# mr3543/3d-Object-Detection

Measured on AMD Instinct MI355X. Metric: lidar sweeps/sec end-to-end fwd (pillarize+backbone), 60k pts, 500×500 BEV, higher is better.
Workload: dtype f32

## Files before the change

### 3d-object-detection_amd/csrc/pp_conv_split.hip

```cpp

#include <algorithm>

#include "pp_conv_split.h"
#include "pp_conv_train.h"
#include "pp_conv_split_tile.h"

namespace pp {

namespace {

using G = TileGeo<8, 1, 1, 2>;

}

template <bool BARE>
__global__ __launch_bounds__(256, 1) void k_conv3x3_split(const float *__restrict__ x,
                                                          const uint4 *__restrict__ w,
                                                          const float *__restrict__ esc,
                                                          const float *__restrict__ prm,
                                                          float *__restrict__ y, int H, int W, int Cin,
                                                          int64_t y_stride, int tiles_x, int tiles_y) {
  __shared__ __attribute__((aligned(16))) unsigned char lds[2 * G::kBufBytes];

  const int lane = threadIdx.x & 63, wave = threadIdx.x >> 6;
  int bx, by, b;
  tile_of_block(tiles_x, tiles_y, bx, by, b);
  const int oy0 = by * G::kRows, ox0 = bx * kTw;
  const int co0 = blockIdx.y * kCo;
  const int nchunks = Cin / kKc;
  Stager<G, BARE> stage(x, w, b, H, W, Cin, oy0 - 1, ox0 - 1, nchunks);
  if constexpr (BARE) stage.xs = prm ? prm[0] : 1.0f;

  const int h = lane >> 5, l32 = lane & 31;
  const int a_off = h * G::kAPlane + (2 * wave * G::kHw + l32) * 16;
  const int b_off = G::kABytes + (h * kCo + l32) * 16;

  f32x16 m00 = {}, m01 = {}, m10 = {}, m11 = {}, c00 = {}, c01 = {}, c10 = {}, c11 = {};

  auto mfmas = [&](const unsigned char *cur) {
#pragma unroll
    for (int dy = 0; dy < 3; ++dy)
#pragma unroll
      for (int dx = 0; dx < 3; ++dx) {
        const int tap = 3 * dy + dx;
        const unsigned char *pa = cur + a_off + (dy * G::kHw + dx) * 16;
        const unsigned char *pb = cur + b_off + tap * (2 * kCo * 16);
        const f16x8 a0h = *reinterpret_cast<const f16x8 *>(pa);
        const f16x8 a1h = *reinterpret_cast<const f16x8 *>(pa + G::kHw * 16);
        const f16x8 b0h = *reinterpret_cast<const f16x8 *>(pb);
        const f16x8 b1h = *reinterpret_cast<const f16x8 *>(pb + 32 * 16);
        const f16x8 b0l = *reinterpret_cast<const f16x8 *>(pb + G::kBPart);
        const f16x8 b1l = *reinterpret_cast<const f16x8 *>(pb + G::kBPart + 32 * 16);
        const f16x8 a0l = *reinterpret_cast<const f16x8 *>(pa + G::kAPart);
        const f16x8 a1l = *reinterpret_cast<const f16x8 *>(pa + G::kAPart + G::kHw * 16);
        m00 = __builtin_amdgcn_mfma_f32_32x32x16_f16(a0h, b0h, m00, 0, 0, 0);
        m01 = __builtin_amdgcn_mfma_f32_32x32x16_f16(a0h, b1h, m01, 0, 0, 0);
        m10 = __builtin_amdgcn_mfma_f32_32x32x16_f16(a1h, b0h, m10, 0, 0, 0);
        m11 = __builtin_amdgcn_mfma_f32_32x32x16_f16(a1h, b1h, m11, 0, 0, 0);
        c00 = __builtin_amdgcn_mfma_f32_32x32x16_f16(a0h, b0l, c00, 0, 0, 0);
        c01 = __builtin_amdgcn_mfma_f32_32x32x16_f16(a0h, b1l, c01, 0, 0, 0);
        c10 = __builtin_amdgcn_mfma_f32_32x32x16_f16(a1h, b0l, c10, 0, 0, 0);
        c11 = __builtin_amdgcn_mfma_f32_32x32x16_f16(a1h, b1l, c11, 0, 0, 0);
        c00 = __builtin_amdgcn_mfma_f32_32x32x16_f16(a0l, b0h, c00, 0, 0, 0);
        c01 = __builtin_amdgcn_mfma_f32_32x32x16_f16(a0l, b1h, c01, 0, 0, 0);
        c10 = __builtin_amdgcn_mfma_f32_32x32x16_f16(a1l, b0h, c10, 0, 0, 0);
        c11 = __builtin_amdgcn_mfma_f32_32x32x16_f16(a1l, b1h, c11, 0, 0, 0);
      }
  };

  chunk_pipeline(stage, lds, nchunks, mfmas);

  const int co = co0 + l32;
  const float e0 = esc[co], e1 = esc[co + 32];
  const auto ep = [&] {
    if constexpr (BARE)
      return Unscale{prm ? prm[1] : 1.0f};
    else
      return Epilogue<2>(prm, co);
  }();
#pragma unroll
  for (int m = 0; m < 2; ++m) {
    const int oy = oy0 + 2 * wave + m;
    if (oy >= H) continue;
    float *yrow = y + (((int64_t)b * H + oy) * W + ox0) * y_stride + co;
    const f32x16 v0 = m ? m10 : m00, v1 = m ? m11 : m01, d0 = m ? c10 : c00, d1 = m ? c11 : c01;
#pragma unroll
    for (int r = 0; r < 16; ++r) {
      const int px = (r & 3) + 8 * (r >> 2) + 4 * h;
      if (ox0 + px < W) {
        float *yp = yrow + px * y_stride;
        yp[0] = split_output<BARE>(v0[r], d0[r], e0, ep, 0);
        yp[32] = split_output<BARE>(v1[r], d1[r], e1, ep, 1);
      }
    }
  }
}

}

using namespace pp;

template <bool BARE>
static int conv3x3_split(const char *fn, pp_ctx_t *ctx, void *stream_, const float *x_dev, int batch, int height,
                         int width, int in_channels, const void *w_split_dev, int out_channels, const float *prm,
                         float *y_dev, int64_t y_channels, int64_t y_channel_offset) {
  if (int rc = check_conv_f16_args(fn, ctx, x_dev, w_split_dev, BARE ? x_dev : prm, y_dev, batch, height, width,
                                   in_channels, out_channels, y_channels, y_channel_offset))
    return rc;
  const int64_t tiles_x = (width + kTw - 1) / kTw, tiles_y = (height + G::kRows - 1) / G::kRows;
  const int64_t blocks = (int64_t)batch * tiles_x * tiles_y;
  if (blocks > 0x7fffffff ||
      (int64_t)batch * height * width * std::max<int64_t>(in_channels, y_channels) > ((int64_t)1 << 40)) {
    set_error("%s: tensor too large", fn);
    return PP_ERR_VALUE;
  }
  const uint4 *w = static_cast<const uint4 *>(w_split_dev);
  const float *esc = split_scales(w_split_dev, out_channels, in_channels);
  return launch_on_device(ctx, "k_conv3x3_split", [&] {
    hipLaunchKernelGGL(k_conv3x3_split<BARE>, dim3((unsigned)blocks, (unsigned)(out_channels / 64)), dim3(256), 0,
                       static_cast<hipStream_t>(stream_), x_dev, w, esc, prm, y_dev + y_channel_offset, height, width,
                       in_channels, y_channels, (int)tiles_x, (int)tiles_y);
  });
}

extern "C" int pp_conv3x3_split_nhwc_dev(pp_ctx_t *ctx, void *stream_, const float *x_dev, int batch,
                                         int height, int width, int in_channels, const void *w_split_dev,
                                         int out_channels, const float *params_dev, float *y_dev,
                                         int64_t y_channels, int64_t y_channel_offset) {
  return conv3x3_split<false>("pp_conv3x3_split_nhwc_dev", ctx, stream_, x_dev, batch, height, width, in_channels,
                              w_split_dev, out_channels, params_dev, y_dev, y_channels, y_channel_offset);
}

extern "C" int pp_conv3x3_split_bare_nhwc_dev(pp_ctx_t *ctx, void *stream_, const float *x_dev, int batch,
                                              int height, int width, int in_channels, const void *w_split_dev,
                                              int out_channels, const float *x_scale_dev, float *y_dev,
                                              int64_t y_channels, int64_t y_channel_offset) {
  if (reinterpret_cast<uintptr_t>(x_scale_dev) & 3) {
    set_error("pp_conv3x3_split_bare_nhwc_dev: x_scale_dev is not 4-byte aligned");
    return PP_ERR_VALUE;
  }
  return conv3x3_split<true>("pp_conv3x3_split_bare_nhwc_dev", ctx, stream_, x_dev, batch, height, width,
                             in_channels, w_split_dev, out_channels, x_scale_dev, y_dev, y_channels,
                             y_channel_offset);
}
```

Before: 2357.

## Make split conv3x3 persistent with software-pipelined loads interleaved among MFMAs

Turns the split-precision 3x3 conv kernel into a persistent kernel whose grid is capped at the compute-unit count, so each block walks over (tile, output-group) items. Each step interleaves the 108 MFMAs with LDS fragment reads, direct global-to-LDS weight DMA, and the f32→f16 hi/lo conversion of the next chunk's activations, and it prefetches the next item's first chunk while the current item finishes. This is meant to hide load latency and launch/tail costs that the previous one-block-per-tile pipeline exposed. In exchange it relies on hand-written inline asm, explicit vmcnt waits and sched barriers, which are fragile. With one block per CU it may also leave less latency hiding across blocks.

Result: faster. 2556, median of 6 (+8.4%).

```diff
diff --git a/3d-object-detection_amd/csrc/pp_conv_split.hip b/3d-object-detection_amd/csrc/pp_conv_split.hip
--- a/3d-object-detection_amd/csrc/pp_conv_split.hip
+++ b/3d-object-detection_amd/csrc/pp_conv_split.hip
@@ -1,5 +1,7 @@
 
 #include <algorithm>
+#include <type_traits>
+#include <utility>
 
 #include "pp_conv_split.h"
 #include "pp_conv_train.h"
@@ -10,6 +12,130 @@
 namespace {
 
 using G = TileGeo<8, 1, 1, 2>;
+
+typedef __attribute__((address_space(3))) void *lptr_t;
+typedef float f32x4 __attribute__((ext_vector_type(4)));
+typedef unsigned u32x4 __attribute__((ext_vector_type(4)));
+typedef _Float16 f16x2 __attribute__((ext_vector_type(2)));
+
+constexpr int kTapMfmas = 12;
+constexpr int kStepMfmas = 9 * kTapMfmas;
+constexpr int kElems = 8 * G::kNItem;
+constexpr int kFirstSlot = kStepMfmas - 2 * kElems - 1;
+constexpr int kWavePieces = G::kWVecs / 64 / 4;
+static_assert(G::kWVecs % 256 == 0 && kFirstSlot >= kTapMfmas, "whole pieces; the conversion fits in a step");
+
+template <int... I, class F>
+__device__ __forceinline__ void static_for_impl(std::integer_sequence<int, I...>, F &&f) {
+  (f(std::integral_constant<int, I>{}), ...);
+}
+template <int N, class F>
+__device__ __forceinline__ void static_for(F &&f) {
+  static_for_impl(std::make_integer_sequence<int, N>{}, f);
+}
+
+struct Item {
+  int b, oy0, ox0, group;
+  __device__ __forceinline__ Item(int item, int groups, int tiles_x, int tiles_y) {
+    group = item % groups;
+    const int tile = item / groups;
+    ox0 = tile % tiles_x * kTw;
+    const int rest = tile / tiles_x;
+    oy0 = rest % tiles_y * G::kRows;
+    b = rest / tiles_y;
+  }
+};
+
+__device__ __forceinline__ void dma_piece(const uint4 *src, unsigned dst, unsigned lane16) {
+  unsigned keep;
+  asm volatile("s_mov_b32 %0, m0\n\ts_mov_b32 m0, %2\n\ts_nop 0\n\tglobal_load_lds_dwordx4 %1, %3\n\ts_mov_b32 m0, %0"
+               : "=&s"(keep)
+               : "v"(lane16), "s"(dst), "s"(src)
+               : "memory");
+}
+
+template <bool XS>
+struct SplitLoader {
+  static constexpr int kN = G::kNItem;
+  const int tid = threadIdx.x;
+  float xs = 1.0f;
+  const float *xb;
+  int xoff[kN], adst[kN];
+  bool xin[kN];
+  const bool last_item = tid + 256 * (kN - 1) < G::kItems;
+  f32x4 xr[kN][2];
+  u32x4 vh[kN], vl[kN];
+  unsigned eh, el;
+
+  __device__ __forceinline__ SplitLoader() {
+#pragma unroll
+    for (int k = 0; k < kN; ++k) {
+      const int i = tid + 256 * k;
+      const int pix = i >> 1, hy = pix / G::kHw;
+      adst[k] = (i & 1) * G::kAPlane + G::slot(pix, hy, pix - hy * G::kHw) * 16;
+    }
+  }
+
+  __device__ __forceinline__ void place(const float *x, const Item &it, int H, int W, int Cin) {
+    xb = x + (int64_t)it.b * H * W * Cin;
+#pragma unroll
+    for (int k = 0; k < kN; ++k) {
+      const int i = tid + 256 * k;
+      const int pix = i >> 1, hh = i & 1;
+      const int hy = pix / G::kHw, hx = pix - hy * G::kHw;
+      const int iy = it.oy0 - G::kHl + hy, ix = it.ox0 - G::kHl + hx;
+      xin[k] = i < G::kItems && iy >= 0 && iy < H && ix >= 0 && ix < W;
+      xoff[k] = (xin[k] ? (iy * W + ix) * Cin : 0) + 8 * hh;
+    }
+  }
+
+  __device__ __forceinline__ void load(int chunk) {
+    const float *xc = xb + chunk * kKc;
+#pragma unroll
+    for (int k = 0; k < kN; ++k) {
+      const float *p = xc + xoff[k];
+      asm volatile("global_load_dwordx4 %0, %2, off\n\tglobal_load_dwordx4 %1, %2, off offset:16"
+                   : "=&v"(xr[k][0]), "=&v"(xr[k][1])
+                   : "v"(p)
+                   : "memory");
+    }
+  }
+
+  template <int K, int kYounger>
+  __device__ __forceinline__ void arrived() {
+    asm volatile("s_waitcnt vmcnt(%2)" : "+v"(xr[K][0]), "+v"(xr[K][1]) : "n"(kYounger + 2 * (kN - 1 - K)));
+  }
+
+  template <int K, int J>
+  __device__ __forceinline__ void convert() {
+    asm volatile("" : "+v"(xr[K][J >> 2]));
+    float a = xr[K][J >> 2][J & 3];
+    if constexpr (XS) a = a * xs;
+    const _Float16 ah = (_Float16)a, al = (_Float16)((a - (float)ah) * 2048.0f);
+    if constexpr (J % 2 == 0) {
+      eh = __builtin_bit_cast(unsigned short, ah);
+      el = __builtin_bit_cast(unsigned short, al);
+      asm volatile("" : "+v"(eh), "+v"(el));
+    } else {
+      unsigned uh = eh | (unsigned)__builtin_bit_cast(unsigned short, ah) << 16;
+      unsigned ul = el | (unsigned)__builtin_bit_cast(unsigned short, al) << 16;
+      asm volatile("" : "+v"(uh), "+v"(ul));
+      vh[K][J >> 1] = uh;
+      vl[K][J >> 1] = ul;
+    }
+  }
+
+  template <int K>
+  __device__ __forceinline__ void write(unsigned char *buf) const {
+    u32x4 r = vl[K], v = vh[K];
+    if (!xin[K]) r = u32x4{};
+    if (!xin[K]) v = u32x4{};
+    if (K + 1 < kN || last_item) {
+      *reinterpret_cast<u32x4 *>(buf + G::kAPart + adst[K]) = r;
+      *reinterpret_cast<u32x4 *>(buf + adst[K]) = v;
+    }
+  }
+};
 
 }
 
@@ -19,80 +145,164 @@
                                                           const float *__restrict__ esc,
                                                           const float *__restrict__ prm,
                                                           float *__restrict__ y, int H, int W, int Cin,
-                                                          int64_t y_stride, int tiles_x, int tiles_y) {
+                                                          int64_t y_stride, int tiles_x, int tiles_y, int groups,
+                                                          int items) {
   __shared__ __attribute__((aligned(16))) unsigned char lds[2 * G::kBufBytes];
 
-  const int lane = threadIdx.x & 63, wave = threadIdx.x >> 6;
-  int bx, by, b;
-  tile_of_block(tiles_x, tiles_y, bx, by, b);
-  const int oy0 = by * G::kRows, ox0 = bx * kTw;
-  const int co0 = blockIdx.y * kCo;
+  const int lane = threadIdx.x & 63, wave = __builtin_amdgcn_readfirstlane(threadIdx.x >> 6);
   const int nchunks = Cin / kKc;
-  Stager<G, BARE> stage(x, w, b, H, W, Cin, oy0 - 1, ox0 - 1, nchunks);
-  if constexpr (BARE) stage.xs = prm ? prm[0] : 1.0f;
+  const int walk = gridDim.x;
+  int item = blockIdx.x;
+
+  SplitLoader<BARE> ld;
+  float inv = 1.0f;
+  if constexpr (BARE)
+    if (prm) {
+      ld.xs = prm[0];
+      inv = prm[1];
+    }
 
   const int h = lane >> 5, l32 = lane & 31;
   const int a_off = h * G::kAPlane + (2 * wave * G::kHw + l32) * 16;
   const int b_off = G::kABytes + (h * kCo + l32) * 16;
 
-  f32x16 m00 = {}, m01 = {}, m10 = {}, m11 = {}, c00 = {}, c01 = {}, c10 = {}, c11 = {};
-
-  auto mfmas = [&](const unsigned char *cur) {
-#pragma unroll
-    for (int dy = 0; dy < 3; ++dy)
-#pragma unroll
-      for (int dx = 0; dx < 3; ++dx) {
-        const int tap = 3 * dy + dx;
-        const unsigned char *pa = cur + a_off + (dy * G::kHw + dx) * 16;
-        const unsigned char *pb = cur + b_off + tap * (2 * kCo * 16);
-        const f16x8 a0h = *reinterpret_cast<const f16x8 *>(pa);
-        const f16x8 a1h = *reinterpret_cast<const f16x8 *>(pa + G::kHw * 16);
-        const f16x8 b0h = *reinterpret_cast<const f16x8 *>(pb);
-        const f16x8 b1h = *reinterpret_cast<const f16x8 *>(pb + 32 * 16);
-        const f16x8 b0l = *reinterpret_cast<const f16x8 *>(pb + G::kBPart);
-        const f16x8 b1l = *reinterpret_cast<const f16x8 *>(pb + G::kBPart + 32 * 16);
-        const f16x8 a0l = *reinterpret_cast<const f16x8 *>(pa + G::kAPart);
-        const f16x8 a1l = *reinterpret_cast<const f16x8 *>(pa + G::kAPart + G::kHw * 16);
-        m00 = __builtin_amdgcn_mfma_f32_32x32x16_f16(a0h, b0h, m00, 0, 0, 0);
-        m01 = __builtin_amdgcn_mfma_f32_32x32x16_f16(a0h, b1h, m01, 0, 0, 0);
-        m10 = __builtin_amdgcn_mfma_f32_32x32x16_f16(a1h, b0h, m10, 0, 0, 0);
-        m11 = __builtin_amdgcn_mfma_f32_32x32x16_f16(a1h, b1h, m11, 0, 0, 0);
-        c00 = __builtin_amdgcn_mfma_f32_32x32x16_f16(a0h, b0l, c00, 0, 0, 0);
-        c01 = __builtin_amdgcn_mfma_f32_32x32x16_f16(a0h, b1l, c01, 0, 0, 0);
-        c10 = __builtin_amdgcn_mfma_f32_32x32x16_f16(a1h, b0l, c10, 0, 0, 0);
-        c11 = __builtin_amdgcn_mfma_f32_32x32x16_f16(a1h, b1l, c11, 0, 0, 0);
-        c00 = __builtin_amdgcn_mfma_f32_32x32x16_f16(a0l, b0h, c00, 0, 0, 0);
-        c01 = __builtin_amdgcn_mfma_f32_32x32x16_f16(a0l, b1h, c01, 0, 0, 0);
-        c10 = __builtin_amdgcn_mfma_f32_32x32x16_f16(a1l, b0h, c10, 0, 0, 0);
-        c11 = __builtin_amdgcn_mfma_f32_32x32x16_f16(a1l, b1h, c11, 0, 0, 0);
-      }
+  f32x16 acc[8];
+  f16x8 fr[2][8];
+
+  const unsigned lds_addr = (unsigned)(uintptr_t)(lptr_t)lds;
+  const unsigned lane16 = lane * 16;
+  const int wpiece0 = G::kABytes + wave * (kWavePieces * 1024);
+  auto wpieces = [&](int group, int chunk) {
+    return w + ((int64_t)group * nchunks + chunk) * G::kWVecs + wave * (kWavePieces * 64);
   };
 
-  chunk_pipeline(stage, lds, nchunks, mfmas);
-
-  const int co = co0 + l32;
-  const float e0 = esc[co], e1 = esc[co + 32];
-  const auto ep = [&] {
-    if constexpr (BARE)
-      return Unscale{prm ? prm[1] : 1.0f};
+  auto read_frag = [&](const unsigned char *cur, auto tap_, auto f_) __attribute__((always_inline)) {
+    constexpr int tap = decltype(tap_)::value, f = decltype(f_)::value;
+    constexpr int a = (tap / 3 * G::kHw + tap % 3) * 16, b = tap * (2 * kCo * 16);
+    constexpr int off = f == 0 ? a : f == 1 ? a + G::kHw * 16 : f == 2 ? b : f == 3 ? b + 32 * 16 : f == 4 ? b + G::kBPart
+                        : f == 5 ? b + G::kBPart + 32 * 16 : f == 6 ? a + G::kAPart : a + G::kAPart + G::kHw * 16;
+    fr[tap & 1][f] = *reinterpret_cast<const f16x8 *>(cur + ((f < 2 || f >= 6) ? a_off : b_off) + off);
+  };
+
+  int par = 0;
+  auto step = [&](int ngroup, int nchunk, auto first_, auto more_) __attribute__((always_inline)) {
+    constexpr bool first = decltype(first_)::value, more = decltype(more_)::value;
+    const unsigned char *cur = lds + par * G::kBufBytes;
+    unsigned char *nxt = lds + (par ^ 1) * G::kBufBytes;
+    static_for<8>([&](auto f) { read_frag(cur, std::integral_constant<int, 0>{}, f); });
+    if constexpr (more) ld.load(nchunk);
+    const uint4 *wsrc = wpieces(ngroup, nchunk);
+    const unsigned wdst = lds_addr + (par ^ 1) * G::kBufBytes + wpiece0;
+    __builtin_amdgcn_sched_barrier(0);
+    static_for<kStepMfmas>([&](auto m_) {
+      constexpr int m = decltype(m_)::value, tap = m / kTapMfmas, i = m % kTapMfmas, s = tap & 1;
+      constexpr int ia = (i < 8 ? 0 : 6) + ((i >> 1) & 1), ib = (i >= 4 && i < 8 ? 4 : 2) + (i & 1);
+      constexpr int ic = (i < 4 ? 0 : 4) + (i & 3);
+      if constexpr (first && m < 8)
+        acc[ic] = __builtin_amdgcn_mfma_f32_32x32x16_f16(fr[s][ia], fr[s][ib], f32x16{}, 0, 0, 0);
+      else
+        acc[ic] = __builtin_amdgcn_mfma_f32_32x32x16_f16(fr[s][ia], fr[s][ib], acc[ic], 0, 0, 0);
+      __builtin_amdgcn_sched_barrier(0);
+      if constexpr (tap + 1 < 9 && i < 8) {
+        read_frag(cur, std::integral_constant<int, tap + 1>{}, std::integral_constant<int, i>{});
+        __builtin_amdgcn_sched_barrier(0);
+      }
+      if constexpr (more && m < kWavePieces) {
+        dma_piece(wsrc + m * 64, wdst + m * 1024, lane16);
+        __builtin_amdgcn_sched_barrier(0);
+      }
+      if constexpr (more && m >= kFirstSlot) {
+        constexpr int j = m - kFirstSlot, e = j / 2;
+        if constexpr (j % 2 == 0 && e < kElems) {
+          if constexpr (e % 8 == 0) ld.template arrived<e / 8, kWavePieces>();
+          ld.template convert<e / 8, e % 8>();
+          __builtin_amdgcn_sched_barrier(0);
+        } else if constexpr (j % 2 == 1 && e % 8 == 7 && e < kElems) {
+          ld.template write<e / 8>(nxt);
+          __builtin_amdgcn_sched_barrier(0);
+        }
+      }
+    });
+    if constexpr (more) __builtin_amdgcn_s_waitcnt(kWaitVm0);
+    __syncthreads();
+    par ^= 1;
+  };
+
+  auto finish = [&](const Item &it) __attribute__((always_inline)) {
+    const int co = it.group * kCo + l32;
+    const float e0 = esc[co], e1 = esc[co + 32];
+    const auto ep = [&] {
+      if constexpr (BARE)
+        return Unscale{inv};
+      else
+        return Epilogue<2>(prm, co);
+    }();
+    auto rows = [&](auto whole_) __attribute__((always_inline)) {
+#pragma unroll
+      for (int m = 0; m < 2; ++m) {
+        const int oy = it.oy0 + 2 * wave + m;
+        if (oy >= H) continue;
+        float *yp = y + ((((int64_t)it.b * H + oy) * W + it.ox0) + 4 * h) * y_stride + co;
+        const f32x16 v0 = acc[2 * m], v1 = acc[2 * m + 1], d0 = acc[4 + 2 * m], d1 = acc[4 + 2 * m + 1];
+#pragma unroll
+        for (int r = 0; r < 16; ++r) {
+          const int px = (r & 3) + 8 * (r >> 2);
+          if (decltype(whole_)::value || it.ox0 + px + 4 * h < W) {
+            yp[0] = split_output<BARE>(v0[r], d0[r], e0, ep, 0);
+            yp[32] = split_output<BARE>(v1[r], d1[r], e1, ep, 1);
+          }
+          yp += ((r & 3) == 3 ? 5 : 1) * y_stride;
+        }
+      }
+    };
+    if (it.ox0 + kTw <= W)
+      rows(std::true_type{});
     else
-      return Epilogue<2>(prm, co);
-  }();
-#pragma unroll
-  for (int m = 0; m < 2; ++m) {
-    const int oy = oy0 + 2 * wave + m;
-    if (oy >= H) continue;
-    float *yrow = y + (((int64_t)b * H + oy) * W + ox0) * y_stride + co;
-    const f32x16 v0 = m ? m10 : m00, v1 = m ? m11 : m01, d0 = m ? c10 : c00, d1 = m ? c11 : c01;
-#pragma unroll
-    for (int r = 0; r < 16; ++r) {
-      const int px = (r & 3) + 8 * (r >> 2) + 4 * h;
-      if (ox0 + px < W) {
-        float *yp = yrow + px * y_stride;
-        yp[0] = split_output<BARE>(v0[r], d0[r], e0, ep, 0);
-        yp[32] = split_output<BARE>(v1[r], d1[r], e1, ep, 1);
-      }
-    }
+      rows(std::false_type{});
+  };
+
+  Item it(item, groups, tiles_x, tiles_y);
+  ld.place(x, it, H, W, Cin);
+  ld.load(0);
+  static_for<kWavePieces>([&](auto i) {
+    dma_piece(wpieces(it.group, 0) + decltype(i)::value * 64, lds_addr + wpiece0 + decltype(i)::value * 1024, lane16);
+  });
+  static_for<kElems>([&](auto e_) {
+    constexpr int e = decltype(e_)::value;
+    if constexpr (e % 8 == 0) ld.template arrived<e / 8, kWavePieces>();
+    ld.template convert<e / 8, e % 8>();
+  });
+  static_for<G::kNItem>([&](auto k) { ld.template write<decltype(k)::value>(lds); });
+  __builtin_amdgcn_s_waitcnt(kWaitVm0);
+  __syncthreads();
+
+  constexpr std::true_type yes{};
+  constexpr std::false_type no{};
+  const bool single = nchunks == 1;
+#pragma unroll 1
+  for (;;) {
+    const bool follows = item + walk < items;
+    const Item nit(follows ? item + walk : item, groups, tiles_x, tiles_y);
+    if (single && !follows) {
+      step(0, 0, yes, no);
+    } else {
+      if (single) ld.place(x, nit, H, W, Cin);
+      step(single ? nit.group : it.group, single ? 0 : 1, yes, yes);
+#pragma unroll 1
+      for (int chunk = 1; chunk < nchunks; ++chunk) {
+        const bool last = chunk + 1 == nchunks;
+        if (last && !follows) {
+          step(0, 0, no, no);
+          break;
+        }
+        if (last) ld.place(x, nit, H, W, Cin);
+        step(last ? nit.group : it.group, last ? 0 : chunk + 1, no, yes);
+      }
+    }
+    finish(it);
+    if (!follows) break;
+    it = nit;
+    item += walk;
   }
 }
 
@@ -108,18 +318,19 @@
                                    in_channels, out_channels, y_channels, y_channel_offset))
     return rc;
   const int64_t tiles_x = (width + kTw - 1) / kTw, tiles_y = (height + G::kRows - 1) / G::kRows;
-  const int64_t blocks = (int64_t)batch * tiles_x * tiles_y;
-  if (blocks > 0x7fffffff ||
+  const int64_t groups = out_channels / 64, items = (int64_t)batch * tiles_x * tiles_y * groups;
+  if (items > 0x7fffffff ||
       (int64_t)batch * height * width * std::max<int64_t>(in_channels, y_channels) > ((int64_t)1 << 40)) {
     set_error("%s: tensor too large", fn);
     return PP_ERR_VALUE;
   }
   const uint4 *w = static_cast<const uint4 *>(w_split_dev);
   const float *esc = split_scales(w_split_dev, out_channels, in_channels);
+  const int64_t grid = std::min<int64_t>(items, compute_units(ctx->device));
   return launch_on_device(ctx, "k_conv3x3_split", [&] {
-    hipLaunchKernelGGL(k_conv3x3_split<BARE>, dim3((unsigned)blocks, (unsigned)(out_channels / 64)), dim3(256), 0,
+    hipLaunchKernelGGL(k_conv3x3_split<BARE>, dim3((unsigned)grid), dim3(256), 0,
                        static_cast<hipStream_t>(stream_), x_dev, w, esc, prm, y_dev + y_channel_offset, height, width,
-                       in_channels, y_channels, (int)tiles_x, (int)tiles_y);
+                       in_channels, y_channels, (int)tiles_x, (int)tiles_y, (int)groups, (int)items);
   });
 }
 
```
